# zenlc2000/pycuda-euler

Hardware: AMD Instinct MI355X
Metric: k-mers/sec (encode+hash+deBruijn+Euler), 10Mx100bp k=31, 1/2/4/8 GPU (higher is better)
Workload: dtype u64

## Files before the change

pycuda-euler_amd/csrc/assemble.hip:

```cpp
#include "common.h"
#include "count_global.h"
#include "graph.h"

#include <rocprim/rocprim.hpp>

#include <algorithm>
#include <cmath>
#include <climits>
#include <cstring>
#include <cstddef>
#include <functional>
#include <type_traits>
#include <vector>

#include "count_part.h"
#include "count_v2.h"
#include "count_sk2.h"
#include "shard.h"
#include "compact.h"
#include "count_wide.h"
#include "hostin.h"
#include "join_w.h"
#include "extended.h"
#include "rank_tile.h"
// ... 288 lines not shown
    unsigned int slots = 2048;
};
BucketPlan plan_buckets(double est, long long limit) {
    constexpr int PMAX = 3;
    BucketPlan p;
    const double filt_max = limit >= 1 ? 32768.0 : PART_KEYS * (1 << PMAX);
    p.part = est / FINE <= 2400.0 || est / FINE <= filt_max;
    p.filt = p.part && (est / FINE > 2400.0 || kn().force_filter);
    while (p.pmax < PMAX && est / FINE / (double)(1 << p.pmax) > PART_KEYS) p.pmax++;
    if (kn().filter_pmax) p.pmax = std::max(1, std::min(PMAX, kn().filter_pmax));
    while (p.bbits < FINE_BITS && est / (double)(1ull << p.bbits) > 1100.0) p.bbits++;
    p.slots = p.filt ? (2048u << p.pmax) : est / (double)(1ull << p.bbits) > 1100.0 ? 4096u : 2048u;
    return p;
}

static uint64_t skpart_slots(int npf, int w, bool val) {
    static thread_local int cache[3][SK_W_MAX + 1][2] = {};
    const int ni = npf == 4 ? 0 : npf == 7 ? 1 : 2;
    int &c = cache[ni][w][val];
    if (!c) {
        const void *fn = nullptr;
#define EC_SKF(NPF, W)                                                                                        \
    if (npf == NPF && w == W) fn = val ? (const void *)&k_skpart_w<NPF, W, true> : (const void *)&k_skpart_w<NPF, W, false>;
#define EC_SKF_W(W) EC_SKF(4, W) EC_SKF(7, W) EC_SKF(10, W)
        EC_SKF_W(7) EC_SKF_W(8) EC_SKF_W(9) EC_SKF_W(10) EC_SKF_W(11) EC_SKF_W(12)
        EC_SKF_W(13) EC_SKF_W(14) EC_SKF_W(15) EC_SKF_W(16) EC_SKF_W(17) EC_SKF_W(18)
#undef EC_SKF_W
#undef EC_SKF
        int dev = 0, ncu = 0, per = 0;
        if (!fn || hipGetDevice(&dev) != hipSuccess ||
            hipDeviceGetAttribute(&ncu, hipDeviceAttributeMultiprocessorCount, dev) != hipSuccess ||
            hipOccupancyMaxActiveBlocksPerMultiprocessor(&per, fn, PT_THREADS, 0) != hipSuccess || per < 1)
            return 1;
        c = ncu * per;
    }
    return (uint64_t)c;
}

int phase_count_sk2(ec_session *s, const uint8_t *d_reads, const uint64_t *d_off, uint64_t nreads,
                    uint64_t read_base, int k, long long limit, uint32_t M, uint64_t G, uint64_t gsize, uint64_t P,
                    int npf, unsigned int &U, SolidIndex &sidx, bool &done, bool validate = false,
                    bool *invalid = nullptr) {
    done = false;
    if (invalid) *invalid = false;
    if (k >= SK_MIN_K && k <= 32) {
        const uint64_t ntiles = (nreads + 63) / 64, slots = skpart_slots(npf, k - SK_M + 1, validate);
        uint64_t g = std::max<uint64_t>(1, std::min<uint64_t>(ntiles, RF_MAX_RUNS));
        if (g > slots) g = g / slots * slots;
        gsize = ((ntiles + g - 1) / g) * 64;
        G = (nreads + gsize - 1) / gsize;
    }
    if (k < SK_MIN_K || k > 32 || M > 256 || gsize * M >= (1ull << 24) || (read_base + nreads) * 2 * M >= (1ull << 32) ||
        kn().no_sk2)
        return EC_OK;
    hipStream_t st = s->stream;
    Scalars *dsc = s->scal.as<Scalars>();
    Scalars hsc;
    auto reset = [&]() -> int {
        if (validate) {
            EC_HIP(hipMemsetAsync(dsc, 0, sizeof(Scalars), st));
            EC_HIP(hipMemsetAsync(&dsc->bad, 0xFF, sizeof(unsigned long long), st));
// ... 8 lines not shown
    const MinCfg mc = sk_cfg(k);
    constexpr uint64_t C = 1ull << SK2_CBITS;
    const double per_read = 2.0 * M / (mc.w + 1) + 2.0;
    const uint64_t cap = (uint64_t)(gsize * per_read * 1.4 / C) + 256;
    EC_CHECK(s->recs.ensure((C * G * cap + SK2_ECAP_W) * 16));
    EC_CHECK(s->cnt.ensure(C * G * 4));
    EC_CHECK(s->hll.ensure(G * (1 << HLL_REG_BITS)));
    EC_CHECK(s->ftot.ensure((1 << HLL_REG_BITS) * 4));
    uint4 *recs = s->recs.as<uint4>();
    const uint32_t smask = P >= (1ull << 26) ? 255u : 0u;
    unsigned int *hreg = s->ftot.as<unsigned int>();
    if (!validate) EC_HIP(hipMemsetAsync(&dsc->nrec, 0, sizeof(unsigned long long), st));
    mark(s, 2 * EC_STAGE_COUNT);
    kmark(s, 1, 0);
#define EC_SKPART_WV(NPF, W, VAL)                                                                             \
    k_skpart_w<NPF, W, VAL><<<lgb - lga, PT_THREADS, 0, st>>>(                                                   \
        d_reads, d_off, nreads, mc, M, gsize, (uint32_t)G, cap, smask, recs, s->cnt.as<unsigned int>(),          \
        s->hll.as<uint8_t>(), &dsc->nrec, &dsc->overflow, &dsc->lens[2], &dsc->npos, lga, elim)
#define EC_SKPART_W(NPF, W)            \
    if (validate)                      \
        EC_SKPART_WV(NPF, W, true);    \
    else                               \
        EC_SKPART_WV(NPF, W, false)
#define EC_SKPART_NPF(W)              \
    if (npf == 4) EC_SKPART_W(4, W);  \
    else if (npf == 7) EC_SKPART_W(7, W); \
    else EC_SKPART_W(10, W)
    const bool chunked = s->pipe.active && s->pipe.done < s->pipe.nchunks;
    if (!chunked) EC_CHECK(pipe_all(s));
    unsigned lga = 0, lgb = (unsigned)G;
    const uint32_t elim = kn().sk2_elim >= 128 ? (uint32_t)std::min(kn().sk2_elim, SK2_ECAP_W) : (uint32_t)SK2_ECAP_W;
    for (int pc = chunked ? 0 : s->pipe.nchunks; ; pc++) {
      if (chunked) {
        if (pc >= s->pipe.nchunks) break;
        lgb = pc + 1 == s->pipe.nchunks ? (unsigned)G : (unsigned)std::min<uint64_t>(G, s->pipe.ravail[pc] / gsize);
        if (lgb <= lga) continue;
        EC_CHECK(pipe_upto(s, pc));
      }
      {
        switch (mc.w) {
            case 7: EC_SKPART_NPF(7); break;
            case 8: EC_SKPART_NPF(8); break;
            case 9: EC_SKPART_NPF(9); break;
            case 10: EC_SKPART_NPF(10); break;
            case 11: EC_SKPART_NPF(11); break;
            case 12: EC_SKPART_NPF(12); break;
            case 13: EC_SKPART_NPF(13); break;
            case 14: EC_SKPART_NPF(14); break;
            case 15: EC_SKPART_NPF(15); break;
            case 16: EC_SKPART_NPF(16); break;
            case 17: EC_SKPART_NPF(17); break;
            default: EC_SKPART_NPF(18); break;
        }
      }
      if (!chunked) break;
      lga = lgb;
    }
#undef EC_SKPART_NPF
#undef EC_SKPART_W
#undef EC_SKPART_WV
    kmark(s, 1, 1);
    EC_HIP(hipMemsetAsync(hreg, 0, (1 << HLL_REG_BITS) * 4, st));
    k_hll_merge<<<dim3((1 << HLL_REG_BITS) / 256, TOT_SLICES), 256, 0, st>>>(s->hll.as<uint8_t>(), G, hreg);
    k_hll_final<<<1, 1024, 0, st>>>(hreg, HLL_REG_BITS, &dsc->est);
    EC_CHECK(d2h(s, &hsc, dsc, sizeof(Scalars), st));
    auto launch_refine = [&](int bb, uint64_t fc) -> int {
// ... 4603 lines not shown
```

pycuda-euler_amd/csrc/count_sk2.h:

```cpp
#pragma once
#include "count_v2.h"
#include "superkmer.h"

namespace ec {

constexpr int SK2_NMAX = 16;
constexpr int SK2_ECAP_W = 1024;
constexpr int SK2_FLUSH_AT = SK2_ECAP_W - 64 - 640;
#ifndef SK2_PD_DEF
#define SK2_PD_DEF 4
#endif
constexpr int SK2_PD = SK2_PD_DEF;
constexpr int SK2_HQ = 128;
constexpr int SK2_BASES = 46;
#ifndef SK2_TILE_DEF
#define SK2_TILE_DEF 2048
#endif
constexpr int SK2_TILE = SK2_TILE_DEF;
constexpr int SK2_CBITS = 6;
constexpr int SK2_BBITS = 14;
constexpr int SK2_FBITS = SK2_BBITS - SK2_CBITS;

__host__ __device__ constexpr inline uint32_t sk2_nmax(int k) {
    return (uint32_t)(SK2_BASES - k + 1 < SK2_NMAX ? SK2_BASES - k + 1 : SK2_NMAX);
}

__device__ inline uint32_t sk_bases16(const uint32_t *st, uint32_t p) {
    return __builtin_amdgcn_alignbit(st[(p >> 4) + 1], st[p >> 4], 2 * (p & 15));
}
__device__ inline void sk_hll_put(unsigned int *s_hll, uint32_t hh) {
    const uint32_t hj = hh >> (32 - HLL_REG_BITS);
    const uint32_t rho = (uint32_t)__clz((int)((hh << HLL_REG_BITS) | (1u << (HLL_REG_BITS - 1)))) + 1;
    const uint32_t hs = (hj & 3) * 8;
    uint32_t old = s_hll[hj >> 2];
    while (rho > ((old >> hs) & 0xFFu)) {
        const uint32_t nw = (old & ~(0xFFu << hs)) | (rho << hs);
        const uint32_t prev = atomicCAS(&s_hll[hj >> 2], old, nw);
        if (prev == old) break;
        old = prev;
    }
}

template <int C>
__device__ inline void skpart_flush(uint32_t cntw, const uint32_t *ent, uint16_t *srt, unsigned int *wcnt,
                                    unsigned int *cur, unsigned long long *base, const uint32_t *rel,
                                    const uint32_t *st, uint32_t lane, unsigned long long gcap, uint64_t cap,
                                    unsigned long long spill, uint32_t M, uint32_t rtile, uint4 *recs,
                                    unsigned int *overflow, unsigned int *s_hll, uint32_t *hq, uint32_t smaskb,
                                    int k, uint64_t kmask) {
    wave_sync();
    for (uint32_t i = lane; i < cntw; i += 64) atomicAdd(&wcnt[ent[i] >> 26], 1u);
    wave_sync();
    const unsigned int v = lane < (uint32_t)C ? wcnt[lane] : 0u;
    const unsigned int incl = wave_incl_scan(v);
    const unsigned int beg = incl - v;
    if (lane < (uint32_t)C) {
        wcnt[lane] = beg;
        unsigned int at = 0;
// ... 20 lines not shown
                const uint32_t p = (qe & 0xFFFFu) + q;
                const uint64_t K = (uint64_t)sk_bases16(st, p) | (uint64_t)sk_bases16(st, p + 16) << 32;
                const uint64_t krc = ~K & kmask, kfw = rev2_64(K) >> (64 - 2 * k);
                sk_hll_put(s_hll, (uint32_t)(mix64(kfw < krc ? kfw : krc) >> 32));
            }
        }
        wave_sync();
        nq = 0;
    };
    for (uint32_t i0 = 0; i0 < cntw; i0 += 64) {
        const uint32_t i = i0 + lane;
        bool samp = false;
        uint32_t qv = 0;
        if (i < cntw) {
            const uint32_t e = ent[srt[i]];
            const uint32_t lr = e & 63u, w0 = (e >> 6) & 0xFFu, n1 = (e >> 14) & 15u;
            const uint32_t p0 = rel[lr] + w0;
            uint4 o;
            o.x = sk_bases16(st, p0);
            o.y = sk_bases16(st, p0 + 16);
            o.z = (sk_bases16(st, p0 + 32) & 0x0FFFFFFFu) | n1 << 28;
            o.w = ((e >> 18) & ((1u << SK2_FBITS) - 1)) << 24 | ((rtile + lr) * M + w0);
            recs[base[e >> 26] + i] = o;
            samp = ((e >> 18) & smaskb) == 0;
            qv = p0 | n1 << 16;
        }
        const uint64_t sb = __builtin_amdgcn_ballot_w64(samp);
        if (samp) hq[nq + __builtin_amdgcn_mbcnt_hi((uint32_t)(sb >> 32), __builtin_amdgcn_mbcnt_lo((uint32_t)sb, 0u))] = qv;
        nq += (uint32_t)__popcll(sb);
        if (nq > (uint32_t)(SK2_HQ - 64)) hll_drain();
    }
    if (nq) hll_drain();
    wave_sync();
    if (lane < (uint32_t)C) wcnt[lane] = 0;
}

template <int NPF, int W, bool VAL>
__global__ void __launch_bounds__(PT_THREADS) k_skpart_w(const uint8_t *__restrict__ buf,
                                                         const uint64_t *__restrict__ off, uint64_t nreads, MinCfg mc,
                                                         uint32_t M, uint64_t gsize, uint32_t G, uint64_t cap,
                                                         uint32_t smask, uint4 *recs, unsigned int *cnt, uint8_t *hll,
                                                         unsigned long long *nrec, unsigned int *overflow,
                                                         unsigned int *vfail, unsigned long long *npos,
                                                         uint32_t g_lo, uint32_t elim) {
    constexpr int C = 1 << SK2_CBITS;
    constexpr int NREG = 1 << HLL_REG_BITS;
    constexpr int SW = NPF * 64 + 4;
    static_assert(SK2_FLUSH_AT >= 64, "the entry buffer holds a flush's worth");
    __shared__ uint32_t s_stage[PT_WAVES][SW];
    __shared__ uint32_t s_ent[PT_WAVES][SK2_ECAP_W];
    __shared__ uint16_t s_srt[PT_WAVES][SK2_ECAP_W];
    __shared__ uint32_t s_rel[PT_WAVES][64];
    __shared__ unsigned long long s_base[PT_WAVES][C];
    __shared__ unsigned int s_wcnt[PT_WAVES][C];
    __shared__ unsigned int s_cur[C];
    __shared__ unsigned int s_hll[NREG / 4];
    __shared__ uint32_t s_hq[PT_WAVES][SK2_HQ];
    const uint32_t lane = threadIdx.x & 63;
    const uint32_t wid = __builtin_amdgcn_readfirstlane(threadIdx.x >> 6);
    for (int i = threadIdx.x; i < NREG / 4; i += PT_THREADS) s_hll[i] = 0;
    if (threadIdx.x < C) s_cur[threadIdx.x] = 0;
    if (lane < C) s_wcnt[wid][lane] = 0;
    __syncthreads();
    const uint64_t g = blockIdx.x + (uint64_t)g_lo;
    const uint64_t g0 = min(g * gsize, nreads), g1 = min(g0 + gsize, nreads);
    const uint32_t ntile = (uint32_t)((g1 - g0 + 63) / 64);
    const int k = mc.k;
    constexpr uint32_t nmax = sk2_nmax(W + SK_M - 1);
    const uint64_t kmask = kmask64(k);
    uint4 pf[NPF];
    uint64_t nx_base = 0;
    uint32_t nx_s = 0, nx_e = 0, nx_n = 0, nx_lo = 0, nx_hi = 0, nx_n16 = 0;
    uint32_t nwin = 0;
    if (wid < ntile) EC_PT_ISSUE(wid);
    const unsigned long long gcap = g * C * cap, spill = (unsigned long long)C * G * cap;
    uint32_t *st = s_stage[wid];
    uint32_t *ent = s_ent[wid];
    for (uint32_t t = wid; t < ntile; t += PT_WAVES) {
        if (VAL) {
            uint32_t diff = 0;
#pragma unroll
            for (int q = 0; q < NPF; q++) {
                const uint32_t wv[4] = {pf[q].x, pf[q].y, pf[q].z, pf[q].w};
// ... 52 lines not shown
#pragma unroll
            for (int tb = 0; tb < m - 1; tb++) push_base(tb < 16 ? (x0 >> (2 * tb)) & 3u : (x1 >> (2 * (tb - 16))) & 3u);
#pragma unroll
            for (int j = 0; j < W; j++) {
                const int tb = m - 1 + j;
                push_base(tb < 16 ? (x0 >> (2 * tb)) & 3u : (x1 >> (2 * (tb - 16))) & 3u);
                S[j] = mmer_hash(mf < mr ? mf : mr);
            }
#pragma unroll
            for (int j = W - 2; j >= 0; j--) S[j] = min(S[j], S[j + 1]);
        }
        const uint32_t nrounds = __any(has) ? (M + W - 1) / W : 0u;
        uint32_t runv = S[0], rsx = 0, cntw = 0;
        const uint64_t hasm = __builtin_amdgcn_ballot_w64(has);
        const uint32_t rtile = 64 * t;
        auto entry = [&](uint32_t end) { return (runv << 18) + lane + (((end - 1u) << 14) + rsx); };
        auto rs_term = [](uint32_t w) { return (uint32_t)((int)w * -16320); };
        for (uint32_t round = 0; round < nrounds; round++) {
            const uint32_t w0 = round * W;
            const uint32_t q = rel + w0 + W;
            const uint32_t a0 = sk_bases16(st, q), a1 = sk_bases16(st, q + 16);
            const uint32_t rw0 = rs_term(w0);
            uint32_t H[W];
            uint32_t P = 0xFFFFFFFFu;
            auto window = [&](int j) {
                const uint32_t v = min(S[j], P);
                const int tb = m - 1 + j;
                const uint32_t b = tb < 16 ? (a0 >> (2 * tb)) & 3u : (a1 >> (2 * (tb - 16))) & 3u;
                mf = (mf << 2) | b;
                const uint32_t fw = mf & MMASK;
                const uint32_t le = j == 0 ? a0 : j < 16 ? __builtin_amdgcn_alignbit(a1, a0, 2 * j) : a1 >> (2 * (j - 16));
                const uint32_t rc = ~le & MMASK;
                H[j] = mmer_hash(fw < rc ? fw : rc);
                P = min(P, H[j]);
                const uint32_t end = w0 + j;
                const bool c1 = v != runv, c2 = rsx == rw0 + (uint32_t)((j - (int)nmax) * -16320);
                const bool close = has & (c1 | c2);
                const uint64_t bal = (__builtin_amdgcn_ballot_w64(c1) | __builtin_amdgcn_ballot_w64(c2)) & hasm;
                if (close) {
                    const uint32_t rk = __builtin_amdgcn_mbcnt_hi((uint32_t)(bal >> 32),
                                                                  __builtin_amdgcn_mbcnt_lo((uint32_t)bal, 0u));
                    ent[min(cntw, elim - 64) + rk] = entry(end);
                    rsx = rw0 + (uint32_t)(j * -16320);
                }
                cntw += (uint32_t)__popcll(bal);
                runv = v;
            };
            if (w0 + W <= M) {
#pragma unroll
                for (int j = 0; j < W; j++) window(j);
            } else {
#pragma unroll
                for (int j = 0; j < W; j++) {
                    if (w0 + j >= M) break;
                    window(j);
                }
            }
#pragma unroll
            for (int j = 0; j < W; j++) S[j] = H[j];
#pragma unroll
            for (int j = W - 2; j >= 0; j--) S[j] = min(S[j], S[j + 1]);
            if (cntw > elim - 64) {
                if (lane == 0) atomicOr(overflow, 1u);
                cntw = elim - 64;
            }
            if (round + 1 < nrounds && cntw > elim - 64 - 640) {
                skpart_flush<C>(cntw, ent, s_srt[wid], s_wcnt[wid], s_cur, s_base[wid], s_rel[wid], st, lane, gcap,
                                cap, spill, M, rtile, recs, overflow, s_hll, s_hq[wid], smask ? 0xFFu : 0u, k,
                                kmask);
                cntw = 0;
            }
        }
        EC_PT_ISSUE(more ? t + PT_WAVES : t);
        if (nrounds) {
            const uint64_t bal = hasm;
            if (has) {
                const uint32_t rk = __builtin_amdgcn_mbcnt_hi((uint32_t)(bal >> 32),
                                                              __builtin_amdgcn_mbcnt_lo((uint32_t)bal, 0u));
                ent[cntw + rk] = entry(M);
            }
            cntw += (uint32_t)__popcll(bal);
            skpart_flush<C>(cntw, ent, s_srt[wid], s_wcnt[wid], s_cur, s_base[wid], s_rel[wid], st, lane, gcap,
                            cap, spill, M, rtile, recs, overflow, s_hll, s_hq[wid], smask ? 0xFFu : 0u, k, kmask);
        }
    }
    __shared__ unsigned int s_nwin[PT_WAVES];
    if (VAL && lane == 0) s_nwin[wid] = nwin;
    __syncthreads();
    if (threadIdx.x < C) cnt[(uint64_t)threadIdx.x * G + g] = (unsigned int)min((uint64_t)s_cur[threadIdx.x], cap);
    if (threadIdx.x == 0) {
        unsigned long long tot = 0;
        for (int c = 0; c < C; c++) tot += s_cur[c];
        if (tot) atomicAdd(nrec, tot);
        if (VAL) {
            unsigned long long wn = 0;
            for (int q = 0; q < PT_WAVES; q++) wn += s_nwin[q];
            if (wn) atomicAdd(npos, wn * M);
        }
    }
    unsigned int *hw = reinterpret_cast<unsigned int *>(hll + g * NREG);
    for (int i = threadIdx.x; i < NREG / 4; i += PT_THREADS) hw[i] = s_hll[i];
}

__device__ inline uint32_t rev2_32b(uint32_t v) {
    v = __builtin_bitreverse32(v);
    return ((v >> 1) & 0x55555555u) | ((v & 0x55555555u) << 1);
}
__device__ inline bool sk2_canon(uint32_t &r0, uint32_t &r1, uint32_t &r2, int k) {
    const unsigned int n = (r2 >> 28) + 1, L2 = 2 * (n + (unsigned int)k - 1);
    const uint32_t m1 = L2 >= 64 ? 0xFFFFFFFFu : (1u << ((L2 - 32) & 31)) - 1u;
    const uint32_t mw2 = L2 > 64 ? (1u << ((L2 - 64) & 31)) - 1u : 0u;
    const uint32_t x0 = r0, x1 = r1 & m1, x2 = r2 & mw2;
    const uint32_t y0 = rev2_32b(x2), y1 = rev2_32b(x1), y2 = rev2_32b(x0);
    const unsigned int sft = 96 - L2, s5 = sft & 31;
    const bool lo = sft < 32;
    const uint32_t a0 = __builtin_amdgcn_alignbit(y1, y0, s5), a1 = __builtin_amdgcn_alignbit(y2, y1, s5),
                   a2 = y2 >> s5;
    const uint32_t q0 = ~(lo ? a0 : a1), q1 = ~(lo ? a1 : a2) & m1, q2 = lo ? ~a2 & mw2 : 0u;
    const bool flip = q2 != x2 ? q2 < x2 : q1 != x1 ? q1 < x1 : q0 < x0;
    r0 = flip ? q0 : x0, r1 = flip ? q1 : x1, r2 = (flip ? q2 : x2) | (n - 1) << 28;
    return flip;
}
__device__ inline void sk2_events(uint32_t w, unsigned int n, uint32_t M, double inv_m, uint32_t &EA, uint32_t &EB) {
    const unsigned int p = w & 0x7FFFFFFFu;
    const bool flip = (w >> 31) != 0;
    const unsigned int rd0 = (unsigned int)((double)p * inv_m);
    int rm = (int)(p - rd0 * M);
    unsigned int rd = rd0;
    if (rm < 0) rd--, rm += (int)M;
    else if (rm >= (int)M) rd++, rm -= (int)M;
    const unsigned int A = rd * 2 * M + (unsigned int)rm, B = rd * 2 * M + 2 * M - 1 - (unsigned int)rm;
    EA = flip ? B - n + 1 : A, EB = flip ? A + n - 1 : B;
}

__global__ void __launch_bounds__(BUCKET_THREADS) k_skrefine(const uint4 *recs, const unsigned int *cnt, uint32_t G,
// ... 50 lines not shown
                const uint4 v = recs[((ga + jr) * C + c) * cap + (l - lst[jr])];
                rx[q] = v.x, ry[q] = v.y, rz[q] = v.z, rw[q] = v.w;
                lr[q] = jr;
            }
        }
#pragma unroll
        for (int q = 0; q < PER; q++) {
            const unsigned int i = threadIdx.x + q * BUCKET_THREADS;
            if (i < n) {
                jj[q] = fb ? (rw[q] >> 24) >> (SK2_FBITS - fb) : 0u;
                rk[q] = atomicAdd(&tcnt[jj[q]], 1u);
                const uint32_t p = (uint32_t)((read_base + (uint64_t)(ga + lr[q]) * gsize) * M) + (rw[q] & 0xFFFFFFu);
#ifdef SK2_CHECK_P31
                assert((p >> 31) == 0);
#endif
                rw[q] = p | (uint32_t)sk2_canon(rx[q], ry[q], rz[q], k) << 31;
            }
        }
        __syncthreads();
        unsigned long long mybase = 0;
        unsigned int myv = 0;
        if (threadIdx.x < REFINE_FANOUT) {
            const unsigned int v = (int)threadIdx.x < F ? tcnt[threadIdx.x] : 0u;
            unsigned int incl = v;
            for (int o = 1; o < 64; o <<= 1) {
                const unsigned int u = __shfl_up(incl, o);
                if (lane >= o) incl += u;
            }
            tbeg[threadIdx.x] = incl - v;
            if (lane == 63) wsum[wid] = incl;
            myv = v;
// ... 82 lines not shown
    auto phase = [&](int i) {
        if (dbg && tid == 0) {
            const unsigned long long t = wall_clock64();
            if (i) atomicAdd(&dbg[2 + i], t - t_last);
            t_last = t;
        }
    };
    phase(0);
    __syncthreads();
    const uint64_t r0 = bbeg[b], r1 = bend[b];
    const uint64_t kmask = kmask64(k);
    const int sh = 2 * (k - 1), fsh = 64 - 2 * k;

    unsigned long long n_rolled = 0;
    auto roll_out = [&](uint32_t x0, uint32_t x1, uint32_t x2, unsigned int mult, unsigned int ea, unsigned int eb) {
        const unsigned int n = (x2 >> 28) + 1;
        if (dbg) n_rolled += n;
        auto events = [&](uint64_t fwd, uint64_t rc, unsigned int o, unsigned int &eC, unsigned int &eT,
                          unsigned int &add) {
            const bool tw = fwd > rc;
            const unsigned int ef = ea + o, et = eb - o;
            add = mult;
            eC = tw ? et : ef;
            eT = tw ? ef : et;
            if (EVEN_K && fwd == rc) {
                add = 2 * mult;
                eC = eT = min(ef, et);
            }
            return tw ? rc : fwd;
        };
        const unsigned int h = (n + 1) >> 1;
// ... 54 lines not shown
            acc += t - c_t;
            c_t = t;
        }
    };
    if (dbg) c_t = __builtin_amdgcn_s_memtime();
    auto record_round = [&](uint4 (&nxd)[RB], uint64_t c0) {
        if (dbg) n_rounds++;
        uint32_t K0[RB], K1[RB], K2[RB], EA[RB], EB[RB], TG[RB], SL[RB];
        int ST[RB];
#pragma unroll
        for (int j = 0; j < RB; j++) {
            const uint64_t ri = c0 + tid + (uint64_t)j * BUCKET_THREADS;
            const bool valid = ri < r1;
            const uint4 x = nxd[j];
            nxd[j] = recs[min(ri + PD * ROUND, r1 - 1)];
            const unsigned int n = (x.z >> 28) + 1;
            K0[j] = x.x, K1[j] = x.y, K2[j] = x.z;
            sk2_events(x.w, n, M, inv_m, EA[j], EB[j]);
            uint32_t hh = K0[j] * 0x9E3779B1u;
            hh = (hh ^ (hh >> 15) ^ K1[j]) * 0x85EBCA77u;
            hh = (hh ^ (hh >> 13) ^ K2[j]) * 0xC2B2AE3Du;
            hh ^= hh >> 16;
            TG[j] = (hh | 0x1000u) & 0xFFFFF000u;
            SL[j] = __umulhi(hh * 0x27D4EB2Fu, (unsigned int)RS);
            ST[j] = valid ? 0 : 1;
        }
        auto searching = [&]() {
            bool a = false;
#pragma unroll
            for (int j = 0; j < RB; j++) a |= ST[j] == 0;
            return a;
// ... 62 lines not shown
    __syncthreads();
    tick(c_bar);
    if (dbg && (tid & 63) == 0) {
        atomicAdd(&dbg[8], c_canon), atomicAdd(&dbg[9], c_probe), atomicAdd(&dbg[10], c_post);
        atomicAdd(&dbg[11], n_iter), atomicAdd(&dbg[12], c_bar), atomicAdd(&dbg[13], n_rounds);
    }
    phase(2);
    {
        constexpr int PER = (RS + BUCKET_THREADS - 1) / BUCKET_THREADS;
        unsigned int sl[PER], rk[PER];
#pragma unroll
        for (int q = 0; q < PER; q++) {
            const unsigned int i = tid + q * BUCKET_THREADS;
            sl[q] = SK2_NMAX;
            if (i < (unsigned)RS && r_tag[i]) {
                sl[q] = SK2_NMAX - 1 - (r_z[i] >> 28);
                rk[q] = atomicAdd(&s_ncnt[sl[q]], 1u);
            }
        }
        __syncthreads();
        if (tid == 0) {
            unsigned int a = 0;
            for (int q = 0; q < SK2_NMAX; q++) {
                const unsigned int v = s_ncnt[q];
                s_ncnt[q] = a;
                a += v;
            }
            s_ncnt[SK2_NMAX] = a;
            if (dbg) atomicAdd(&dbg[0], (unsigned long long)a), atomicAdd(&dbg[1], 1ull);
        }
        __syncthreads();
// ... 12 lines not shown
        tick(c_roll);
        __syncthreads();
        tick(c_bar2);
        if (dbg && (tid & 63) == 0) atomicAdd(&dbg[14], c_roll), atomicAdd(&dbg[15], c_bar2);
        if (dbg) atomicAdd(&dbg[2], n_rolled);
    }
    phase(4);
    lds_table_finish<SLOTS, false, KeyId>(tab, s_over, b, limit, dkey, dcnt, dfc, dft, sub, nsolid, ndistinct,
                                          overflow, KeyId(), EvExpand{2 * M});
    phase(5);
}


template <int SLOTS, int RS, int NT>
struct SkB3Lds {
    static constexpr int NC = RS / 2;
    struct Rec {
        uint32_t tag[RS], x[RS], y[RS], z[RS], mult[RS], a[RS], b[RS];
    };
    struct Roll {
        LTabE<SLOTS> tab;
        uint32_t x[NC], y[NC], z[NC], mult[NC], a[NC], b[NC];
    };
    union {
        Rec r;
        Roll k;
    };
};

template <int SLOTS, int RS, int NT, bool EVEN_K, bool STATS = false>
__global__ void __launch_bounds__(NT) k_skbucket3(const uint4 *recs, const unsigned long long *bbeg,
                                                  const unsigned long long *bend, int k, uint32_t M, double inv_m,
                                                  long long limit, unsigned long long *dkey, unsigned int *dcnt,
                                                  unsigned long long *dfc, unsigned long long *dft, SubSlot *sub,
                                                  unsigned int *nsolid, unsigned long long *ndistinct,
                                                  unsigned int *overflow, unsigned long long *dbg,
                                                  unsigned int claim_cap, unsigned int *bmark = nullptr) {
    constexpr int SBITS = __builtin_ctz(SLOTS);
    constexpr uint32_t PEND = 0x800u;
    constexpr unsigned int CLAIM_MAX = RS / 2 < RS - 1 - NT ? RS / 2 : RS - 1 - NT;
    static_assert(RS > NT + 1, "record table too small for the records in flight");
    static_assert(sizeof(typename SkB3Lds<SLOTS, RS, NT>::Roll) <= sizeof(typename SkB3Lds<SLOTS, RS, NT>::Rec),
                  "the k-mer table and the compact records fit the record table's space");
    constexpr int OV = 256;
    __shared__ SkB3Lds<SLOTS, RS, NT> L;
    __shared__ uint32_t o_x[OV], o_y[OV], o_z[OV], o_a[OV], o_b[OV];
    __shared__ unsigned int s_over[2];
    __shared__ unsigned int s_nent, s_nov, s_ncnt[SK2_NMAX + 1];
    auto &R = L.r;
    auto &tab = L.k.tab;
    const unsigned int b = blockIdx.x, tid = threadIdx.x;
    for (int i = tid; i < RS; i += NT) {
        R.tag[i] = 0;
        R.mult[i] = 0;
        R.a[i] = R.b[i] = 0xFFFFFFFFu;
    }
    if (tid <= SK2_NMAX) s_ncnt[tid] = 0;
    if (tid == 0) s_over[0] = s_over[1] = 0, s_nent = 0, s_nov = 0;
    __syncthreads();
    const uint64_t r0 = bbeg[b], r1 = bend[b];
    const uint64_t kmask = kmask64(k);
    const int sh = 2 * (k - 1), fsh = 64 - 2 * k;
    unsigned long long n_rolled = 0;

    auto roll_out = [&](uint32_t x0, uint32_t x1, uint32_t x2, unsigned int mult, unsigned int ea, unsigned int eb) {
        const unsigned int n = (x2 >> 28) + 1;
        if (dbg) n_rolled += n;
        auto events = [&](uint64_t fwd, uint64_t rc, unsigned int o, unsigned int &eC, unsigned int &eT,
                          unsigned int &add) {
            const bool tw = fwd > rc;
            const unsigned int ef = ea + o, et = eb - o;
            add = mult;
            eC = tw ? et : ef;
            eT = tw ? ef : et;
            if (EVEN_K && fwd == rc) {
                add = 2 * mult;
                eC = eT = min(ef, et);
            }
            return tw ? rc : fwd;
        };
        const unsigned int h = (n + 1) >> 1;
// ... 44 lines not shown
    unsigned long long c_canon = 0, c_probe = 0, c_post = 0, n_iter = 0, n_rounds = 0, c_t = 0;
    auto tick = [&](unsigned long long &acc) {
        if constexpr (STATS) {
            const unsigned long long t = __builtin_amdgcn_s_memtime();
            acc += t - c_t;
            c_t = t;
        }
    };
    if constexpr (STATS) c_t = __builtin_amdgcn_s_memtime();
    auto record_round = [&](uint4 &nxd, uint64_t c0) {
        if constexpr (STATS) n_rounds++;
        const uint64_t ri = c0 + tid;
        const bool valid = ri < r1;
        const uint4 x = nxd;
        nxd = recs[min(ri + PD * NT, r1 - 1)];
        const unsigned int n = (x.z >> 28) + 1;
        const uint32_t K0 = x.x, K1 = x.y, K2 = x.z;
        uint32_t EA, EB;
        sk2_events(x.w, n, M, inv_m, EA, EB);
        uint32_t hh = K0 * 0x9E3779B1u;
        hh = (hh ^ (hh >> 15) ^ K1) * 0x85EBCA77u;
        hh = (hh ^ (hh >> 13) ^ K2) * 0xC2B2AE3Du;
        hh ^= hh >> 16;
        const uint32_t TG = (hh | 0x1000u) & 0xFFFFF000u;
        uint32_t SL = __umulhi(hh * 0x27D4EB2Fu, (unsigned int)RS);
        int ST = valid ? 0 : 1;
        tick(c_canon);
#pragma unroll 1
        while (__any(ST == 0)) {
            if constexpr (STATS) n_iter++;
            const uint32_t T = ld(&R.tag[SL]);
// ... 43 lines not shown
        unsigned long long c_bar = 0;
        tick(c_bar);
        if ((tid & 63) == 0) {
            atomicAdd(&dbg[8], c_canon), atomicAdd(&dbg[9], c_probe), atomicAdd(&dbg[10], c_post);
            atomicAdd(&dbg[11], n_iter), atomicAdd(&dbg[12], c_bar), atomicAdd(&dbg[13], n_rounds);
        }
    }
    constexpr int PER = (RS + NT - 1) / NT;
    uint32_t cx[PER], cy[PER], cz[PER], cm[PER], ca[PER], cb[PER], bin[PER], rk[PER];
#pragma unroll
    for (int q = 0; q < PER; q++) {
        const unsigned int i = tid + q * NT;
        bin[q] = SK2_NMAX;
        if (i < (unsigned)RS && R.tag[i]) {
            cx[q] = R.x[i], cy[q] = R.y[i], cz[q] = R.z[i], cm[q] = R.mult[i], ca[q] = R.a[i], cb[q] = R.b[i];
            bin[q] = SK2_NMAX - 1 - (cz[q] >> 28);
            rk[q] = atomicAdd(&s_ncnt[bin[q]], 1u);
        }
    }
    __syncthreads();
    if (tid == 0) {
        unsigned int a = 0;
        for (int q = 0; q < SK2_NMAX; q++) {
            const unsigned int v = s_ncnt[q];
            s_ncnt[q] = a;
            a += v;
        }
        s_ncnt[SK2_NMAX] = a;
        if (dbg) {
            atomicAdd(&dbg[0], (unsigned long long)a), atomicAdd(&dbg[1], 1ull);
            atomicMax(&dbg[3], (unsigned long long)(a + min(s_nov, (unsigned int)OV)));
// ... 52 lines not shown
    __shared__ unsigned int seen1[NW], seen2[NW];
    __shared__ unsigned int s_cells[2];
    const unsigned int b = blockIdx.x, tid = threadIdx.x;
    for (int i = tid; i < SLOTS; i += NT) {
        tab.key[i] = EMPTY_KEY;
        tab.count[i] = 0;
        tab.ev[i] = make_uint2(0xFFFFFFFFu, 0xFFFFFFFFu);
    }
    for (unsigned int i = tid; i < NW; i += NT) seen1[i] = seen2[i] = 0;
    if (tid == 0) s_over[0] = s_over[1] = 0, s_cells[0] = s_cells[1] = 0;
    __syncthreads();
    const uint64_t r0 = bbeg[b], r1 = bend[b];
    const uint64_t kmask = kmask64(k);
    const int fsh = 64 - 2 * k;
    auto windows = [&](uint64_t ri, const uint4 &x, auto &&fn) {
        const unsigned int n = (x.z >> 28) + 1;
        uint32_t EA, EB;
        unsigned int mult = 1;
        if constexpr (MERGED) {
            const uint2 e = mev[ri];
            EA = e.x, EB = e.y, mult = x.w;
        } else {
            sk2_events(x.w, n, M, inv_m, EA, EB);
        }
        for (unsigned int o = 0; o < n; o++) {
            const uint32_t lo = __builtin_amdgcn_alignbit(x.y, x.x, 2 * o), hi = __builtin_amdgcn_alignbit(x.z, x.y, 2 * o);
            const uint64_t P = (uint64_t)lo | (uint64_t)hi << 32;
            const uint64_t rv = ~P & kmask, fw = rev2_64(P) >> fsh;
            const bool tw = fw > rv;
            const unsigned int ef = EA + o, et = EB - o;
            unsigned int add = mult, eC = tw ? et : ef, eT = tw ? ef : et;
            if (EVEN_K && fw == rv) {
                add = 2 * mult;
                eC = eT = min(ef, et);
            }
            fn(tw ? rv : fw, add, eC, eT);
        }
    };
    auto cells = [](unsigned long long c, unsigned int &c1, unsigned int &c2) {
        const uint64_t h = mix64(c);
        c1 = (unsigned int)(h >> 12) & CM;
// ... 88 lines not shown
        tag[i] = 0;
        tm[i] = 0;
        ta[i] = tb[i] = 0xFFFFFFFFu;
    }
    if (tid == 0) s_nent = 0, s_nout = 0, s_nrej = 0;
    if (tid < (unsigned int)SK2_NMAX) s_ncnt[tid] = 0;
    __syncthreads();
    const uint64_t r0 = bbeg[b], r1 = bend[b];
    auto ld = [](uint32_t *a) { return __hip_atomic_load(a, __ATOMIC_RELAXED, __HIP_MEMORY_SCOPE_WORKGROUP); };
    uint4 nxt = r1 > r0 ? recs[min(r0 + tid, r1 - 1)] : make_uint4(0u, 0u, 0u, 0u);
    for (uint64_t c0 = r0; c0 < r1; c0 += NT) {
        const uint64_t ri = c0 + tid;
        const bool valid = ri < r1;
        const uint4 x = nxt;
        if (c0 + NT < r1) nxt = recs[min(ri + NT, r1 - 1)];
        const unsigned int n = (x.z >> 28) + 1;
        const uint32_t K0 = x.x, K1 = x.y, K2 = x.z;
        uint32_t EA, EB;
        sk2_events(x.w, n, M, inv_m, EA, EB);
        uint32_t hh = K0 * 0x9E3779B1u;
        hh = (hh ^ (hh >> 15) ^ K1) * 0x85EBCA77u;
        hh = (hh ^ (hh >> 13) ^ K2) * 0xC2B2AE3Du;
        hh ^= hh >> 16;
        const uint32_t TG = (hh | 0x1000u) & 0xFFFFF000u;
        uint32_t SL = __umulhi(hh * 0x27D4EB2Fu, (unsigned int)RS);
        int ST = valid ? 0 : 1;
#pragma unroll 1
        while (__any(ST == 0)) {
            const uint32_t T = ld(&tag[SL]);
            asm volatile("" ::: "memory");
            const uint32_t X = ld(&tx[SL]), Y = ld(&ty[SL]), Z = ld(&tz[SL]);
// ... 24 lines not shown
        if (ST == 2) {
            if (dbg) atomicAdd(&s_nrej, 1u);
            const uint64_t o = r0 + atomicAdd(&s_nout, 1u);
            mrec[o] = make_uint4(K0, K1, K2, 1u);
            mev[o] = make_uint2(EA, EB);
        }
    }
    __syncthreads();
    constexpr int PER = (RS + NT - 1) / NT;
    uint32_t bin[PER], rk[PER];
#pragma unroll
    for (int q = 0; q < PER; q++) {
        const unsigned int i = tid + q * NT;
        bin[q] = SK2_NMAX;
        if (i < (unsigned int)RS && tag[i]) {
            bin[q] = SK2_NMAX - 1 - (tz[i] >> 28);
            rk[q] = atomicAdd(&s_ncnt[bin[q]], 1u);
        }
    }
    __syncthreads();
    if (tid == 0) {
        unsigned int a = s_nout;
        for (int q = 0; q < SK2_NMAX; q++) {
            const unsigned int v = s_ncnt[q];
            s_ncnt[q] = a;
            a += v;
        }
        s_nout = a;
    }
    __syncthreads();
#pragma unroll
// ... 20 lines not shown
```

Before: 204.2 billion.

## Encode super-k-mer length with sentinel bit to allow 17-window runs at k=31

Replaces the 4-bit run-count field in the super-k-mer record's top bits with a sentinel-bit length encoding, which lets runs hold up to 17 k-mers (47 bases). At k=31 with short reads it adds a kernel variant whose entry packing uses a 7-bit window offset and more count bits, so a full 17-wide minimizer window becomes a single record instead of two. Fewer, longer records should shrink partition and count traffic. Decoding now needs a clz per record, and the LDS compact-table sizing changes.

```diff
diff --git a/pycuda-euler_amd/csrc/assemble.hip b/pycuda-euler_amd/csrc/assemble.hip
--- a/pycuda-euler_amd/csrc/assemble.hip
+++ b/pycuda-euler_amd/csrc/assemble.hip
@@ -326,14 +326,18 @@
     return p;
 }
 
-static uint64_t skpart_slots(int npf, int w, bool val) {
-    static thread_local int cache[3][SK_W_MAX + 1][2] = {};
+static uint64_t skpart_slots(int npf, int w, bool val, bool n17) {
+    static thread_local int cache[3][SK_W_MAX + 2][2] = {};
     const int ni = npf == 4 ? 0 : npf == 7 ? 1 : 2;
-    int &c = cache[ni][w][val];
+    int &c = cache[ni][n17 ? SK_W_MAX + 1 : w][val];
     if (!c) {
         const void *fn = nullptr;
+#define EC_SKF17(NPF) \
+    if (n17 && npf == NPF) fn = val ? (const void *)&k_skpart_w<NPF, 17, true, true> : (const void *)&k_skpart_w<NPF, 17, false, true>;
+        EC_SKF17(4) EC_SKF17(7) EC_SKF17(10)
+#undef EC_SKF17
 #define EC_SKF(NPF, W)                                                                                        \
-    if (npf == NPF && w == W) fn = val ? (const void *)&k_skpart_w<NPF, W, true> : (const void *)&k_skpart_w<NPF, W, false>;
+    if (!n17 && npf == NPF && w == W) fn = val ? (const void *)&k_skpart_w<NPF, W, true> : (const void *)&k_skpart_w<NPF, W, false>;
 #define EC_SKF_W(W) EC_SKF(4, W) EC_SKF(7, W) EC_SKF(10, W)
         EC_SKF_W(7) EC_SKF_W(8) EC_SKF_W(9) EC_SKF_W(10) EC_SKF_W(11) EC_SKF_W(12)
         EC_SKF_W(13) EC_SKF_W(14) EC_SKF_W(15) EC_SKF_W(16) EC_SKF_W(17) EC_SKF_W(18)
@@ -355,8 +359,9 @@
                     bool *invalid = nullptr) {
     done = false;
     if (invalid) *invalid = false;
+    const bool n17 = k - SK_M + 1 == 17 && M <= SK2_FW17_MAXM;
     if (k >= SK_MIN_K && k <= 32) {
-        const uint64_t ntiles = (nreads + 63) / 64, slots = skpart_slots(npf, k - SK_M + 1, validate);
+        const uint64_t ntiles = (nreads + 63) / 64, slots = skpart_slots(npf, k - SK_M + 1, validate, n17);
         uint64_t g = std::max<uint64_t>(1, std::min<uint64_t>(ntiles, RF_MAX_RUNS));
         if (g > slots) g = g / slots * slots;
         gsize = ((ntiles + g - 1) / g) * 64;
@@ -395,7 +400,7 @@
     mark(s, 2 * EC_STAGE_COUNT);
     kmark(s, 1, 0);
 #define EC_SKPART_WV(NPF, W, VAL)                                                                             \
-    k_skpart_w<NPF, W, VAL><<<lgb - lga, PT_THREADS, 0, st>>>(                                                   \
+    k_skpart_w<NPF, W, VAL, W == 17 && N17><<<lgb - lga, PT_THREADS, 0, st>>>(                                   \
         d_reads, d_off, nreads, mc, M, gsize, (uint32_t)G, cap, smask, recs, s->cnt.as<unsigned int>(),          \
         s->hll.as<uint8_t>(), &dsc->nrec, &dsc->overflow, &dsc->lens[2], &dsc->npos, lga, elim)
 #define EC_SKPART_W(NPF, W)            \
@@ -419,6 +424,7 @@
         EC_CHECK(pipe_upto(s, pc));
       }
       {
+        constexpr bool N17 = false;
         switch (mc.w) {
             case 7: EC_SKPART_NPF(7); break;
             case 8: EC_SKPART_NPF(8); break;
@@ -430,7 +436,14 @@
             case 14: EC_SKPART_NPF(14); break;
             case 15: EC_SKPART_NPF(15); break;
             case 16: EC_SKPART_NPF(16); break;
-            case 17: EC_SKPART_NPF(17); break;
+            case 17:
+                if (n17) {
+                    constexpr bool N17 = true;
+                    EC_SKPART_NPF(17);
+                } else {
+                    EC_SKPART_NPF(17);
+                }
+                break;
             default: EC_SKPART_NPF(18); break;
         }
       }
diff --git a/pycuda-euler_amd/csrc/count_sk2.h b/pycuda-euler_amd/csrc/count_sk2.h
--- a/pycuda-euler_amd/csrc/count_sk2.h
+++ b/pycuda-euler_amd/csrc/count_sk2.h
@@ -4,7 +4,7 @@
 
 namespace ec {
 
-constexpr int SK2_NMAX = 16;
+constexpr int SK2_NMAX = 17;
 constexpr int SK2_ECAP_W = 1024;
 constexpr int SK2_FLUSH_AT = SK2_ECAP_W - 64 - 640;
 #ifndef SK2_PD_DEF
@@ -12,7 +12,7 @@
 #endif
 constexpr int SK2_PD = SK2_PD_DEF;
 constexpr int SK2_HQ = 128;
-constexpr int SK2_BASES = 46;
+constexpr int SK2_BASES = 47;
 #ifndef SK2_TILE_DEF
 #define SK2_TILE_DEF 2048
 #endif
@@ -21,8 +21,17 @@
 constexpr int SK2_BBITS = 14;
 constexpr int SK2_FBITS = SK2_BBITS - SK2_CBITS;
 
-__host__ __device__ constexpr inline uint32_t sk2_nmax(int k) {
-    return (uint32_t)(SK2_BASES - k + 1 < SK2_NMAX ? SK2_BASES - k + 1 : SK2_NMAX);
+constexpr uint32_t SK2_FW17_MAXM = 128;
+__host__ __device__ constexpr inline uint32_t sk2_nmax(int k, int fw = 8) {
+    const int nb = SK2_BASES - k + 1, nf = 1 << (12 - fw);
+    return (uint32_t)(nb < nf ? (nb < SK2_NMAX ? nb : SK2_NMAX) : (nf < SK2_NMAX ? nf : SK2_NMAX));
+}
+__device__ inline unsigned int sk2_len2(uint32_t y, uint32_t z) {
+    return (z ? 95u : 63u) - (unsigned int)__clz((int)(z ? z : y));
+}
+__device__ inline unsigned int sk2_n(uint32_t y, uint32_t z, int k) { return sk2_len2(y, z) / 2 - (unsigned int)k + 1; }
+__device__ inline unsigned int sk2_bin(uint32_t y, uint32_t z, int k) {
+    return (unsigned int)SK2_NMAX - min(max(sk2_n(y, z, k), 1u), (unsigned int)SK2_NMAX);
 }
 
 __device__ inline uint32_t sk_bases16(const uint32_t *st, uint32_t p) {
@@ -41,7 +50,7 @@
     }
 }
 
-template <int C>
+template <int C, int FW>
 __device__ inline void skpart_flush(uint32_t cntw, const uint32_t *ent, uint16_t *srt, unsigned int *wcnt,
                                     unsigned int *cur, unsigned long long *base, const uint32_t *rel,
                                     const uint32_t *st, uint32_t lane, unsigned long long gcap, uint64_t cap,
@@ -92,12 +101,14 @@
         uint32_t qv = 0;
         if (i < cntw) {
             const uint32_t e = ent[srt[i]];
-            const uint32_t lr = e & 63u, w0 = (e >> 6) & 0xFFu, n1 = (e >> 14) & 15u;
+            const uint32_t lr = e & 63u, w0 = (e >> 6) & ((1u << FW) - 1u), n1 = (e >> (6 + FW)) & ((1u << (12 - FW)) - 1u);
             const uint32_t p0 = rel[lr] + w0;
+            const uint32_t sp = 2 * (n1 + (uint32_t)k) - 32, sbit = 1u << (sp & 31);
+            const uint32_t b1 = sk_bases16(st, p0 + 16), b2 = sk_bases16(st, p0 + 32);
             uint4 o;
             o.x = sk_bases16(st, p0);
-            o.y = sk_bases16(st, p0 + 16);
-            o.z = (sk_bases16(st, p0 + 32) & 0x0FFFFFFFu) | n1 << 28;
+            o.y = sp >= 32 ? b1 : (b1 & (sbit - 1u)) | sbit;
+            o.z = sp >= 32 ? (b2 & (sbit - 1u)) | sbit : 0u;
             o.w = ((e >> 18) & ((1u << SK2_FBITS) - 1)) << 24 | ((rtile + lr) * M + w0);
             recs[base[e >> 26] + i] = o;
             samp = ((e >> 18) & smaskb) == 0;
@@ -113,7 +124,7 @@
     if (lane < (uint32_t)C) wcnt[lane] = 0;
 }
 
-template <int NPF, int W, bool VAL>
+template <int NPF, int W, bool VAL, bool N17 = false>
 __global__ void __launch_bounds__(PT_THREADS) k_skpart_w(const uint8_t *__restrict__ buf,
                                                          const uint64_t *__restrict__ off, uint64_t nreads, MinCfg mc,
                                                          uint32_t M, uint64_t gsize, uint32_t G, uint64_t cap,
@@ -144,7 +155,10 @@
     const uint64_t g0 = min(g * gsize, nreads), g1 = min(g0 + gsize, nreads);
     const uint32_t ntile = (uint32_t)((g1 - g0 + 63) / 64);
     const int k = mc.k;
-    constexpr uint32_t nmax = sk2_nmax(W + SK_M - 1);
+    static_assert(!N17 || W == 17, "17-window runs exist at k = 31 only");
+    constexpr int FW = N17 ? 7 : 8;
+    constexpr int RST = (1 << 6) - (1 << (6 + FW));
+    constexpr uint32_t nmax = sk2_nmax(W + SK_M - 1, FW);
     const uint64_t kmask = kmask64(k);
     uint4 pf[NPF];
     uint64_t nx_base = 0;
@@ -227,8 +241,8 @@
         uint32_t runv = S[0], rsx = 0, cntw = 0;
         const uint64_t hasm = __builtin_amdgcn_ballot_w64(has);
         const uint32_t rtile = 64 * t;
-        auto entry = [&](uint32_t end) { return (runv << 18) + lane + (((end - 1u) << 14) + rsx); };
-        auto rs_term = [](uint32_t w) { return (uint32_t)((int)w * -16320); };
+        auto entry = [&](uint32_t end) { return (runv << 18) + lane + (((end - 1u) << (6 + FW)) + rsx); };
+        auto rs_term = [](uint32_t w) { return (uint32_t)((int)w * RST); };
         for (uint32_t round = 0; round < nrounds; round++) {
             const uint32_t w0 = round * W;
             const uint32_t q = rel + w0 + W;
@@ -247,14 +261,14 @@
                 H[j] = mmer_hash(fw < rc ? fw : rc);
                 P = min(P, H[j]);
                 const uint32_t end = w0 + j;
-                const bool c1 = v != runv, c2 = rsx == rw0 + (uint32_t)((j - (int)nmax) * -16320);
+                const bool c1 = v != runv, c2 = rsx == rw0 + (uint32_t)((j - (int)nmax) * RST);
                 const bool close = has & (c1 | c2);
                 const uint64_t bal = (__builtin_amdgcn_ballot_w64(c1) | __builtin_amdgcn_ballot_w64(c2)) & hasm;
                 if (close) {
                     const uint32_t rk = __builtin_amdgcn_mbcnt_hi((uint32_t)(bal >> 32),
                                                                   __builtin_amdgcn_mbcnt_lo((uint32_t)bal, 0u));
                     ent[min(cntw, elim - 64) + rk] = entry(end);
-                    rsx = rw0 + (uint32_t)(j * -16320);
+                    rsx = rw0 + (uint32_t)(j * RST);
                 }
                 cntw += (uint32_t)__popcll(bal);
                 runv = v;
@@ -278,7 +292,7 @@
                 cntw = elim - 64;
             }
             if (round + 1 < nrounds && cntw > elim - 64 - 640) {
-                skpart_flush<C>(cntw, ent, s_srt[wid], s_wcnt[wid], s_cur, s_base[wid], s_rel[wid], st, lane, gcap,
+                skpart_flush<C, FW>(cntw, ent, s_srt[wid], s_wcnt[wid], s_cur, s_base[wid], s_rel[wid], st, lane, gcap,
                                 cap, spill, M, rtile, recs, overflow, s_hll, s_hq[wid], smask ? 0xFFu : 0u, k,
                                 kmask);
                 cntw = 0;
@@ -293,7 +307,7 @@
                 ent[cntw + rk] = entry(M);
             }
             cntw += (uint32_t)__popcll(bal);
-            skpart_flush<C>(cntw, ent, s_srt[wid], s_wcnt[wid], s_cur, s_base[wid], s_rel[wid], st, lane, gcap,
+            skpart_flush<C, FW>(cntw, ent, s_srt[wid], s_wcnt[wid], s_cur, s_base[wid], s_rel[wid], st, lane, gcap,
                             cap, spill, M, rtile, recs, overflow, s_hll, s_hq[wid], smask ? 0xFFu : 0u, k, kmask);
         }
     }
@@ -319,10 +333,11 @@
     v = __builtin_bitreverse32(v);
     return ((v >> 1) & 0x55555555u) | ((v & 0x55555555u) << 1);
 }
-__device__ inline bool sk2_canon(uint32_t &r0, uint32_t &r1, uint32_t &r2, int k) {
-    const unsigned int n = (r2 >> 28) + 1, L2 = 2 * (n + (unsigned int)k - 1);
-    const uint32_t m1 = L2 >= 64 ? 0xFFFFFFFFu : (1u << ((L2 - 32) & 31)) - 1u;
-    const uint32_t mw2 = L2 > 64 ? (1u << ((L2 - 64) & 31)) - 1u : 0u;
+__device__ inline bool sk2_canon(uint32_t &r0, uint32_t &r1, uint32_t &r2) {
+    const unsigned int L2 = sk2_len2(r1, r2);
+    const uint32_t sbit = 1u << (L2 & 31);
+    const uint32_t m1 = L2 >= 64 ? 0xFFFFFFFFu : sbit - 1u;
+    const uint32_t mw2 = L2 >= 64 ? sbit - 1u : 0u;
     const uint32_t x0 = r0, x1 = r1 & m1, x2 = r2 & mw2;
     const uint32_t y0 = rev2_32b(x2), y1 = rev2_32b(x1), y2 = rev2_32b(x0);
     const unsigned int sft = 96 - L2, s5 = sft & 31;
@@ -331,7 +346,9 @@
                    a2 = y2 >> s5;
     const uint32_t q0 = ~(lo ? a0 : a1), q1 = ~(lo ? a1 : a2) & m1, q2 = lo ? ~a2 & mw2 : 0u;
     const bool flip = q2 != x2 ? q2 < x2 : q1 != x1 ? q1 < x1 : q0 < x0;
-    r0 = flip ? q0 : x0, r1 = flip ? q1 : x1, r2 = (flip ? q2 : x2) | (n - 1) << 28;
+    r0 = flip ? q0 : x0;
+    r1 = (flip ? q1 : x1) | (L2 >= 64 ? 0u : sbit);
+    r2 = (flip ? q2 : x2) | (L2 >= 64 ? sbit : 0u);
     return flip;
 }
 __device__ inline void sk2_events(uint32_t w, unsigned int n, uint32_t M, double inv_m, uint32_t &EA, uint32_t &EB) {
@@ -412,7 +429,7 @@
 #ifdef SK2_CHECK_P31
                 assert((p >> 31) == 0);
 #endif
-                rw[q] = p | (uint32_t)sk2_canon(rx[q], ry[q], rz[q], k) << 31;
+                rw[q] = p | (uint32_t)sk2_canon(rx[q], ry[q], rz[q]) << 31;
             }
         }
         __syncthreads();
@@ -525,7 +542,7 @@
 
     unsigned long long n_rolled = 0;
     auto roll_out = [&](uint32_t x0, uint32_t x1, uint32_t x2, unsigned int mult, unsigned int ea, unsigned int eb) {
-        const unsigned int n = (x2 >> 28) + 1;
+        const unsigned int n = min(sk2_n(x1, x2, k), (unsigned int)SK2_NMAX);
         if (dbg) n_rolled += n;
         auto events = [&](uint64_t fwd, uint64_t rc, unsigned int o, unsigned int &eC, unsigned int &eT,
                           unsigned int &add) {
@@ -610,7 +627,7 @@
             const bool valid = ri < r1;
             const uint4 x = nxd[j];
             nxd[j] = recs[min(ri + PD * ROUND, r1 - 1)];
-            const unsigned int n = (x.z >> 28) + 1;
+            const unsigned int n = sk2_n(x.y, x.z, k);
             K0[j] = x.x, K1[j] = x.y, K2[j] = x.z;
             sk2_events(x.w, n, M, inv_m, EA[j], EB[j]);
             uint32_t hh = K0[j] * 0x9E3779B1u;
@@ -703,7 +720,7 @@
             const unsigned int i = tid + q * BUCKET_THREADS;
             sl[q] = SK2_NMAX;
             if (i < (unsigned)RS && r_tag[i]) {
-                sl[q] = SK2_NMAX - 1 - (r_z[i] >> 28);
+                sl[q] = sk2_bin(r_y[i], r_z[i], k);
                 rk[q] = atomicAdd(&s_ncnt[sl[q]], 1u);
             }
         }
@@ -746,7 +763,7 @@
 
 template <int SLOTS, int RS, int NT>
 struct SkB3Lds {
-    static constexpr int NC = RS / 2;
+    static constexpr int NC = (int)((7 * RS * sizeof(uint32_t) - sizeof(LTabE<SLOTS>)) / (6 * sizeof(uint32_t)));
     struct Rec {
         uint32_t tag[RS], x[RS], y[RS], z[RS], mult[RS], a[RS], b[RS];
     };
@@ -770,7 +787,8 @@
                                                   unsigned int claim_cap, unsigned int *bmark = nullptr) {
     constexpr int SBITS = __builtin_ctz(SLOTS);
     constexpr uint32_t PEND = 0x800u;
-    constexpr unsigned int CLAIM_MAX = RS / 2 < RS - 1 - NT ? RS / 2 : RS - 1 - NT;
+    constexpr int NCR = SkB3Lds<SLOTS, RS, NT>::NC;
+    constexpr unsigned int CLAIM_MAX = NCR < RS - 1 - NT ? NCR : RS - 1 - NT;
     static_assert(RS > NT + 1, "record table too small for the records in flight");
     static_assert(sizeof(typename SkB3Lds<SLOTS, RS, NT>::Roll) <= sizeof(typename SkB3Lds<SLOTS, RS, NT>::Rec),
                   "the k-mer table and the compact records fit the record table's space");
@@ -796,7 +814,7 @@
     unsigned long long n_rolled = 0;
 
     auto roll_out = [&](uint32_t x0, uint32_t x1, uint32_t x2, unsigned int mult, unsigned int ea, unsigned int eb) {
-        const unsigned int n = (x2 >> 28) + 1;
+        const unsigned int n = min(sk2_n(x1, x2, k), (unsigned int)SK2_NMAX);
         if (dbg) n_rolled += n;
         auto events = [&](uint64_t fwd, uint64_t rc, unsigned int o, unsigned int &eC, unsigned int &eT,
                           unsigned int &add) {
@@ -871,7 +889,7 @@
         const bool valid = ri < r1;
         const uint4 x = nxd;
         nxd = recs[min(ri + PD * NT, r1 - 1)];
-        const unsigned int n = (x.z >> 28) + 1;
+        const unsigned int n = sk2_n(x.y, x.z, k);
         const uint32_t K0 = x.x, K1 = x.y, K2 = x.z;
         uint32_t EA, EB;
         sk2_events(x.w, n, M, inv_m, EA, EB);
@@ -945,7 +963,7 @@
         bin[q] = SK2_NMAX;
         if (i < (unsigned)RS && R.tag[i]) {
             cx[q] = R.x[i], cy[q] = R.y[i], cz[q] = R.z[i], cm[q] = R.mult[i], ca[q] = R.a[i], cb[q] = R.b[i];
-            bin[q] = SK2_NMAX - 1 - (cz[q] >> 28);
+            bin[q] = sk2_bin(cy[q], cz[q], k);
             rk[q] = atomicAdd(&s_ncnt[bin[q]], 1u);
         }
     }
@@ -1028,7 +1046,7 @@
     const uint64_t kmask = kmask64(k);
     const int fsh = 64 - 2 * k;
     auto windows = [&](uint64_t ri, const uint4 &x, auto &&fn) {
-        const unsigned int n = (x.z >> 28) + 1;
+        const unsigned int n = min(sk2_n(x.y, x.z, k), (unsigned int)SK2_NMAX);
         uint32_t EA, EB;
         unsigned int mult = 1;
         if constexpr (MERGED) {
@@ -1038,7 +1056,8 @@
             sk2_events(x.w, n, M, inv_m, EA, EB);
         }
         for (unsigned int o = 0; o < n; o++) {
-            const uint32_t lo = __builtin_amdgcn_alignbit(x.y, x.x, 2 * o), hi = __builtin_amdgcn_alignbit(x.z, x.y, 2 * o);
+            const uint32_t lo = o < 16 ? __builtin_amdgcn_alignbit(x.y, x.x, 2 * o) : x.y,
+                           hi = o < 16 ? __builtin_amdgcn_alignbit(x.z, x.y, 2 * o) : x.z;
             const uint64_t P = (uint64_t)lo | (uint64_t)hi << 32;
             const uint64_t rv = ~P & kmask, fw = rev2_64(P) >> fsh;
             const bool tw = fw > rv;
@@ -1157,7 +1176,7 @@
         const bool valid = ri < r1;
         const uint4 x = nxt;
         if (c0 + NT < r1) nxt = recs[min(ri + NT, r1 - 1)];
-        const unsigned int n = (x.z >> 28) + 1;
+        const unsigned int n = sk2_n(x.y, x.z, k);
         const uint32_t K0 = x.x, K1 = x.y, K2 = x.z;
         uint32_t EA, EB;
         sk2_events(x.w, n, M, inv_m, EA, EB);
@@ -1212,7 +1231,7 @@
         const unsigned int i = tid + q * NT;
         bin[q] = SK2_NMAX;
         if (i < (unsigned int)RS && tag[i]) {
-            bin[q] = SK2_NMAX - 1 - (tz[i] >> 28);
+            bin[q] = sk2_bin(ty[i], tz[i], k);
             rk[q] = atomicAdd(&s_ncnt[bin[q]], 1u);
         }
     }
```

New measurement: 213.9 billion (median of 6 runs). +4.8%, better.
